# Newiz430/CellSegmentation

Hardware: AMD Instinct MI355X
Metric: tiles/sec fwd+bwd (ResNet-50 MIL, 299x299) (higher is better)
Workload: dtype bf16; 1 GPU; ResNet-50 tile classifier (train_tile.py --scratch semantics: fwd + CE + full bwd + Adam), bag=64 tiles of 299x299x3 per GPU, freeze_bn=True; tiles_per_gpu=64, parallelism=dp1

## Files before the change

### cellsegmentation_amd/csrc/conv_v2.hip

```cpp
#include "cs_common.h"
#include <stdio.h>
#include <stdlib.h>
#include <utility>

namespace {

typedef int i32x4 __attribute__((ext_vector_type(4)));
typedef unsigned u32x4 __attribute__((ext_vector_type(4)));
constexpr unsigned OOB = 0x80000000u;

struct C2Params {
    const void* src;
    const void* wpk;
    void* dst;
    const float* shift;
    const void* residual;
    unsigned char* bits_out;
    const unsigned char* bits_in;
    float* slab;
    int act;
    int SH, SW, SC, NS;
    int DH, DW, NOUT;
    int Wp, Hp, PW, PH;
    int LW;
    int TH, TWl, tiles_x, tiles_y;
    unsigned n_tiles;
    int stride;
    int gather, GH, GWp;
    unsigned tap_sh[9];
    int lin;
    unsigned chunk_bytes;
    int add_stride, AH, AW;
    unsigned mg_dw, sh_dw, mg_dh, sh_dh, mg_wp, sh_wp, mg_hp, sh_hp;
    int NCC;
    int n_ntiles;
    unsigned M;
    unsigned src_bytes;
    unsigned pix_bytes;
    unsigned wpk_bytes;
};

__device__ __forceinline__ unsigned udivm(unsigned n, unsigned mg, unsigned sh) { return __umulhi(n, mg) >> sh; }

__device__ __forceinline__ i32x4 make_rsrc(const void* base, unsigned bytes) {
    const unsigned long long a = (unsigned long long)base;
    i32x4 r;
    r.x = (int)(unsigned)a;
    r.y = (int)((unsigned)(a >> 32) & 0xffffu);
    r.z = (int)bytes;
    r.w = 0x00020000;
    return r;
}
__device__ __forceinline__ unsigned lds_off(const void* p) { return (unsigned)(size_t)(__attribute__((address_space(3))) const unsigned char*)p; }

template <int N> __device__ __forceinline__ void wait_vm() { asm volatile("s_waitcnt vmcnt(%0)" ::"n"(N)); }
template <int N> __device__ __forceinline__ void wait_vm_mem() { asm volatile("s_waitcnt vmcnt(%0)" ::"n"(N) : "memory"); }
__device__ __forceinline__ void raw_barrier() { asm volatile("s_barrier" ::: "memory"); }

__device__ __forceinline__ void dma_block(const i32x4& rsrc, unsigned lds_dst, unsigned voff, unsigned soff) {
    unsigned tmp;
    asm volatile(
        "s_mov_b32 m0, %1\n\t"
        "s_add_u32 %0, %4, 64\n\t"
        "buffer_load_dwordx4 %2, %3, %4 offen lds\n\t"
        "s_add_u32 m0, %1, 0x400\n\t"
// ... 143 lines not shown
    const unsigned wds[4] = {o.x, o.y, o.z, o.w};
    unsigned t = 0;
#pragma unroll
    for (int i = 0; i < 4; ++i) {
        const unsigned a = ((wds[i] & 0x7fff7fffu) + 0x7fff7fffu) & ~wds[i];
        t |= ((a >> 15) & 0x10001u) << (2 * i);
    }
    return (t | (t >> 15)) & 0xffu;
}
__device__ __forceinline__ unsigned nz_bits8(const uint4& o) {
    const unsigned wds[4] = {o.x, o.y, o.z, o.w};
    const unsigned ones = 0x00010001u;
    unsigned u = 0;
#pragma unroll
    for (int i = 0; i < 4; ++i) {
        unsigned t;
        asm("v_pk_min_u16 %0, %1, %2" : "=v"(t) : "v"(wds[i]), "s"(ones));
        u |= t << (2 * i);
    }
    return (u | (u >> 15)) & 0xffu;
}
struct TileOffs {
    static constexpr bool kPreset = false;
    static constexpr unsigned NONE = 0x7fffff00u;
    unsigned rb, mr, bb, br;
    __device__ __forceinline__ void set(unsigned base, bool ok, unsigned nout, unsigned n_w, unsigned piece, unsigned M) {
        const unsigned lane = threadIdx.x & 63;
        const bool live = ok && base != 0xffffffffu;
        const unsigned m = base + (lane >> 2);
        mr = live ? m : NONE;
        rb = (m * nout + n_w + 8u * piece) * 2u;
        const unsigned mbit = m + 16u * (lane & 1u);
        br = (live && !(lane & 2u)) ? mbit : NONE;
        bb = ((n_w >> 5) * M + mbit) * 4u;
    }
    __device__ __forceinline__ unsigned row(unsigned M, unsigned nout, int i, int q) const {
        const unsigned d = (unsigned)(2 * i + q);
        return mr + 16u * d < M ? rb + d * (32u * nout) : OOB;
    }
    __device__ __forceinline__ unsigned bit(unsigned M, unsigned nout, int i) const {
        return br + 32u * (unsigned)i < M ? bb + (unsigned)i * 128u : OOB;
    }
};
template <int TM> struct TileOffs2D {
    static constexpr bool kPreset = true;
    unsigned ro[TM][2], bo[TM];
    __device__ __forceinline__ void set2d(unsigned n, unsigned y0, unsigned x0, unsigned dh, unsigned dw, unsigned twl, unsigned j0, bool alive,
                                          unsigned nout, unsigned n_w, unsigned piece, unsigned M) {
        const unsigned lane = threadIdx.x & 63, tw1 = (1u << twl) - 1u;
#pragma unroll
        for (int i = 0; i < TM; ++i) {
#pragma unroll
            for (int q = 0; q < 2; ++q) {
                const unsigned j = j0 + 32u * i + 16u * q + (lane >> 2);
                const unsigned y = y0 + (j >> twl), x = x0 + (j & tw1);
                const unsigned m = (n * dh + y) * dw + x;
                ro[i][q] = (alive && y < dh && x < dw) ? (m * nout + n_w + 8u * piece) * 2u : OOB;
            }
            const unsigned jb = j0 + 32u * i + (lane >> 2) + 16u * (lane & 1u);
            const unsigned yb = y0 + (jb >> twl), xb = x0 + (jb & tw1);
            const unsigned mb = (n * dh + yb) * dw + xb;
            bo[i] = (alive && !(lane & 2u) && yb < dh && xb < dw) ? ((n_w >> 5) * M + mb) * 4u : OOB;
        }
    }
    __device__ __forceinline__ unsigned row(unsigned, unsigned, int i, int q) const { return ro[i][q]; }
    __device__ __forceinline__ unsigned bit(unsigned, unsigned, int i) const { return bo[i]; }
};
__device__ __forceinline__ uint4 keep_bits8(const uint4& o, unsigned b) {
    unsigned wds[4] = {o.x, o.y, o.z, o.w};
#pragma unroll
    for (int i = 0; i < 4; ++i) {
        const unsigned m = (b >> (2 * i));
        wds[i] &= (m & 1u) * 0xffffu + (m & 2u) * 0x7fff8000u;
    }
    return make_uint4(wds[0], wds[1], wds[2], wds[3]);
}


__device__ __forceinline__ unsigned compact_add_off(const C2Params& p, unsigned m, unsigned n_w, unsigned piece) {
    const unsigned yall = udivm(m, p.mg_dw, p.sh_dw);
    const unsigned x = m - yall * (unsigned)p.DW;
    const unsigned n = udivm(yall, p.mg_dh, p.sh_dh);
    const unsigned y = yall - n * (unsigned)p.DH;
    const unsigned mc = (n * (unsigned)p.AH + (y >> 1)) * (unsigned)p.AW + (x >> 1);
    return (m < p.M && !((x | y) & 1u)) ? (mc * (unsigned)p.NOUT + n_w + 8u * piece) * 2u : OOB;
}
template <bool DG> __device__ __forceinline__ void load_shift(const C2Params& p, int n_w, bool alive, float (&sh)[16]) {
    const int lane = threadIdx.x & 63;
    const int hh = lane >> 5;
#pragma unroll
// ... 72 lines not shown
    }
    __device__ __forceinline__ unsigned acc_lds(int j) const {
        const int lane = threadIdx.x & 63;
        return scr + (unsigned)(lane & 31) * EPI_ROW + (unsigned)(2 * j + (lane >> 5)) * 16u;
    }

    __device__ __forceinline__ unsigned res_off(int i, int q) const {
        if constexpr (TO::kPreset) return to.row(p.M, (unsigned)p.NOUT, i, q);
        else {
            if (p.add_stride <= 1) return to.row(p.M, (unsigned)p.NOUT, i, q);
            const unsigned lane = threadIdx.x & 63;
            const unsigned m = to.mr + 16u * (unsigned)(2 * i + q);
            const unsigned yall = udivm(m, p.mg_dw, p.sh_dw);
            const unsigned x = m - yall * (unsigned)p.DW;
            const unsigned n = udivm(yall, p.mg_dh, p.sh_dh);
            const unsigned y = yall - n * (unsigned)p.DH;
            const unsigned mc = (n * (unsigned)p.AH + (y >> 1)) * (unsigned)p.AW + (x >> 1);
            return (m < p.M && !((x | y) & 1u)) ? (mc * (unsigned)p.NOUT + (unsigned)n_w + 8u * (lane & 3u)) * 2u : OOB;
        }
    }

    __device__ __forceinline__ void prefetch() {
        const int lane = threadIdx.x & 63;
        const unsigned out_bytes = p.M * (unsigned)p.NOUT * 2u;
        if constexpr (!TO::kPreset) to.set(m0w, alive, (unsigned)p.NOUT, (unsigned)n_w, (unsigned)(lane & 3), p.M);
        r_dst = __builtin_amdgcn_make_buffer_rsrc(p.dst, 0, out_bytes, 0x00020000);
        r_res = __builtin_amdgcn_make_buffer_rsrc(const_cast<void*>(p.residual), 0,
                                                  !p.residual ? 0u : p.add_stride == 2 ? (unsigned)(p.NS * p.AH * p.AW * p.NOUT) * 2u : out_bytes, 0x00020000);
        r_bin = __builtin_amdgcn_make_buffer_rsrc(const_cast<unsigned char*>(p.bits_in), 0, p.bits_in ? out_bytes >> 4 : 0u, 0x00020000);
        r_bout = __builtin_amdgcn_make_buffer_rsrc(p.bits_out, 0, p.bits_out ? out_bytes >> 4 : 0u, 0x00020000);
        load_shift<DG>(p, n_w, alive, sh);
#pragma unroll
        for (int i = 0; i < TM; ++i) {
            if constexpr (PRE_RES) {
                rr[i][0] = __builtin_bit_cast(uint4, __builtin_amdgcn_raw_buffer_load_b128(r_res, res_off(i, 0), 0, 0));
                rr[i][1] = __builtin_bit_cast(uint4, __builtin_amdgcn_raw_buffer_load_b128(r_res, res_off(i, 1), 0, 0));
            }
            if constexpr (DG) mb[i] = __builtin_amdgcn_raw_buffer_load_b32(r_bin, to.bit(p.M, (unsigned)p.NOUT, i), 0, 0);
        }
    }

    template <int I> __device__ __forceinline__ void operator()(const f32x16& acc) {
        const int lane = threadIdx.x & 63;
        const unsigned piece = (unsigned)(lane & 3);
        float v[16];
#pragma unroll
        for (int r = 0; r < 16; ++r) v[r] = DG ? acc[r] : acc[r] + sh[r];
// ... 35 lines not shown
        if (!DG && p.bits_out) {
            unsigned w0, w1;
            plane_dwords(o0, o1, p.act == CS_ACT_RELU, piece, w0, w1);
            __builtin_amdgcn_raw_buffer_store_b32((lane & 1) ? w1 : w0, r_bout, to.bit(p.M, (unsigned)p.NOUT, I), 0, 0);
        }
    }

    __device__ __forceinline__ void finish() {
        if (!DG || !p.slab || !alive) return;
        const int lane = threadIdx.x & 63;
#pragma unroll
        for (int k = 0; k < 8; ++k) {
#pragma unroll
            for (int off = 32; off >= 4; off >>= 1) s1[k] += __shfl_xor(s1[k], off, 64);
        }
        if (lane < 4) {
            float* dst = p.slab + (size_t)slab_row * 2 * p.NOUT + n_w + 8 * lane;
            *reinterpret_cast<float4*>(dst) = make_float4(s1[0], s1[1], s1[2], s1[3]);
            *reinterpret_cast<float4*>(dst + 4) = make_float4(s1[4], s1[5], s1[6], s1[7]);
        }
    }
};

template <int NTAP, int SK, int TM, int WM, int WN, int NBW, bool DG, bool T2D = false>
__global__ __launch_bounds__(256, 2) __attribute__((amdgpu_num_vgpr(50))) void conv2_halo_kernel(C2Params p) {
    static_assert(WM * WN == 4 && NTAP % 3 == 0 && NBW <= 8, "layout");
    constexpr int BM = WM * TM * 32, BN = WN * 32;
    constexpr unsigned STAGE = NBW * 4 * 2048;
    extern __shared__ __attribute__((aligned(16))) unsigned char smem[];

    const int tid = threadIdx.x, lane = tid & 63;
    const int wave = __builtin_amdgcn_readfirstlane(tid >> 6);
    const int wm = wave / WN, wn = wave % WN;
    const int l31 = lane & 31, hh = lane >> 5;

    const WgTile wg(p);
    const unsigned mtile = wg.mtile, m0 = mtile * BM;
    if (T2D ? mtile >= p.n_tiles : m0 >= p.M) return;
    const int n_w = wg.n_w(p, BN, wn);
    const bool alive = n_w < p.NOUT;

    using TOffs = std::conditional_t<T2D, TileOffs2D<TM>, TileOffs>;
    Epilogue<TM, (NBW == 8), DG, TOffs> epi(p, m0 + (unsigned)(wm * TM * 32), n_w, mtile * WM + wm, alive, 0u);
    unsigned qb[TM];
    unsigned voff[NBW];
    if constexpr (T2D) {
        const unsigned per_img = (unsigned)(p.tiles_y * p.tiles_x);
        const unsigned n = mtile / per_img, tr = mtile - n * per_img;
        const unsigned ty = tr / (unsigned)p.tiles_x, tx = tr - ty * (unsigned)p.tiles_x;
        const unsigned y0 = ty * (unsigned)p.TH, x0 = tx << p.TWl;
        const unsigned j0 = (unsigned)(wm * TM * 32);
#pragma unroll
        for (int i = 0; i < TM; ++i) {
            const unsigned j = j0 + 32u * i + (unsigned)l31;
            qb[i] = (j >> p.TWl) * (unsigned)p.LW + (j & ((1u << p.TWl) - 1u));
        }
        const unsigned win_rows = (unsigned)(p.TH + (NTAP / SK) - 1) * (unsigned)p.LW;
#pragma unroll
        for (int j = 0; j < NBW; ++j) {
            const unsigned l = 16u * (unsigned)(wave + 4 * j) + (unsigned)(lane & 15);
            const unsigned ly = udivm(l, p.mg_wp, p.sh_wp);
            const unsigned lx = l - ly * (unsigned)p.LW;
            const int sy = (int)(y0 + ly) - p.PH, sx = (int)(x0 + lx) - p.PW;
            const bool real = l < win_rows && (unsigned)sy < (unsigned)p.SH && (unsigned)sx < (unsigned)p.SW;
            const unsigned pix = (n * (unsigned)p.SH + (unsigned)sy) * (unsigned)p.SW + (unsigned)sx;
            voff[j] = real ? pix * p.pix_bytes + (unsigned)(lane >> 4) * 16u : OOB;
        }
        epi.to.set2d(n, y0, x0, (unsigned)p.DH, (unsigned)p.DW, (unsigned)p.TWl, j0, alive, (unsigned)p.NOUT, (unsigned)n_w, (unsigned)(lane & 3), p.M);
    } else {
        auto pos0 = [&](unsigned m) -> unsigned {
            const unsigned yall = udivm(m, p.mg_dw, p.sh_dw);
            const unsigned x = m - yall * (unsigned)p.DW;
            const unsigned n = udivm(yall, p.mg_dh, p.sh_dh);
            const unsigned y = yall - n * (unsigned)p.DH;
            return (n * (unsigned)p.Hp + y) * (unsigned)p.Wp + x;
        };
        const unsigned Lmin = pos0(m0);
        const unsigned m0w = m0 + (unsigned)(wm * TM * 32);
#pragma unroll
        for (int i = 0; i < TM; ++i) {
            unsigned m = m0w + 32u * i + (unsigned)l31;
            if (m > p.M - 1) m = p.M - 1;
            qb[i] = pos0(m) - Lmin;
        }
#pragma unroll
        for (int j = 0; j < NBW; ++j) {
            const unsigned L = Lmin + 16u * (unsigned)(wave + 4 * j) + (unsigned)(lane & 15);
            const unsigned row = udivm(L, p.mg_wp, p.sh_wp);
            const unsigned col = L - row * (unsigned)p.Wp;
            const unsigned n = udivm(row, p.mg_hp, p.sh_hp);
            const unsigned ry = row - n * (unsigned)p.Hp;
            const bool real = col >= (unsigned)p.PW && ry >= (unsigned)p.PH && n < (unsigned)p.NS;
            const unsigned pix = (n * (unsigned)p.SH + (ry - (unsigned)p.PH)) * (unsigned)p.SW + (col - (unsigned)p.PW);
            voff[j] = real ? pix * p.pix_bytes + (unsigned)(lane >> 4) * 16u : OOB;
        }
    }
    const i32x4 rsrc_a = make_rsrc(p.src, p.src_bytes);
    const i32x4 rsrc_b = make_rsrc(p.wpk, p.wpk_bytes);
    const unsigned bvoff = alive ? (unsigned)lane * 16u : OOB;
    unsigned wsoff = (unsigned)(n_w >> 5) * (unsigned)p.NCC * (unsigned)(NTAP * 4096);
    const unsigned smem_base = lds_off(smem);

    static_assert(TM >= 2 && TM <= 4, "the register map of the main loop holds up to 4 pixel tiles per wave");
    epi.prefetch();
    own_registers();
    vzero_seq(std::make_integer_sequence<int, 16 * TM>{});
    const unsigned hhb = (unsigned)hh * 256u;
    const unsigned cf0 = 0xf0u;

#pragma unroll
    for (int j = 0; j < NBW; ++j) dma_block(rsrc_a, smem_base + (unsigned)(wave + 4 * j) * 2048u, voff[j], 0u);
    bload4<0>(rsrc_b, bvoff, wsoff); wsoff += 4096u;
    bload4<1>(rsrc_b, bvoff, wsoff); wsoff += 4096u;
    wait_vm<8>();
    raw_barrier();

    unsigned nxt_soff = 128u;

    auto tap = [&]<int T, bool ODD, bool HN>() {
        constexpr int CUR = T % 3, NX2 = (T + 2) % 3;
        constexpr bool has1 = HN || (T + 1 < NTAP);
        constexpr bool has2 = HN || (T + 2 < NTAP);
        constexpr bool LAST = T == NTAP - 1;
        constexpr int D0 = (HN && !LAST && T < NBW) ? 2 : 0;
        constexpr int D1 = (HN && !LAST && T >= 1 && T - 1 < NBW) ? 2 : 0;
        constexpr int D2 = (HN && !LAST && T >= 2 && T - 2 < NBW) ? 2 : 0;
        constexpr unsigned CUR_STAGE = ODD ? STAGE : 0u, NXT_STAGE = ODD ? 0u : STAGE;
        if constexpr (has2) {
            bload4<NX2>(rsrc_b, bvoff, wsoff);
            wsoff += 4096u;
        }
        if constexpr (D0) dma_block(rsrc_a, smem_base + NXT_STAGE + (unsigned)(wave + 4 * T) * 2048u, voff[T < NBW ? T : 0], nxt_soff);
        wait_vm<(has1 ? 4 : 0) + (has2 ? 4 : 0) + D0 + D1 + D2>();
        const unsigned sh_cur = (unsigned)(T / SK) * (unsigned)p.LW + (unsigned)(T % SK);
        const unsigned sh_next = (unsigned)((T + 1) / SK) * (unsigned)p.LW + (unsigned)((T + 1) % SK);
        if constexpr (T == NTAP - 1 && !HN) epi.scr = smem_base + NXT_STAGE + (unsigned)wave * EPI_WAVE;
        tap_mfma<TM, CUR, T & 1, CUR_STAGE, CUR_STAGE, T == 0, T != NTAP - 1, false, (T == NTAP - 1 && !HN)>(qb[0], qb[1], qb[2 % TM], qb[3 % TM], sh_cur, sh_next,
                                                                                                          hhb, cf0, epi);
    };
    auto chunk = [&]<bool ODD, bool HN>() {
        [&]<int... Ts>(std::integer_sequence<int, Ts...>) { (tap.template operator()<Ts, ODD, HN>(), ...); }(std::make_integer_sequence<int, NTAP>{});
    };

    if constexpr (NBW == 8) {
        chunk.template operator()<false, false>();
    } else {
        for (int cc = 0; cc < p.NCC; cc += 2) {
            if (cc) { raw_barrier(); nxt_soff += 128u; }
            if (cc + 1 < p.NCC) chunk.template operator()<false, true>();
            else chunk.template operator()<false, false>();
            if (cc + 1 < p.NCC) {
                raw_barrier();
                nxt_soff += 128u;
                if (cc + 2 < p.NCC) chunk.template operator()<true, true>();
                else chunk.template operator()<true, false>();
            }
        }
    }
    epi.finish();
}


constexpr int W_TMP = 100, W_AD = 104, W_AF = 120, W_B = 184, W_ACC = 128, W_NSLOT = 18;

template <int N, typename F> __device__ __forceinline__ void for_n(F&& f) {
    [&]<int... Is>(std::integer_sequence<int, Is...>) { (f.template operator()<Is>(), ...); }(std::make_integer_sequence<int, N>{});
}
template <int REG> __device__ __forceinline__ void azero() { asm volatile("v_accvgpr_write_b32 a[%c0], 0" ::"i"(REG)); }
template <int REG> __device__ __forceinline__ float aget() {
    float x;
    asm volatile("v_accvgpr_read_b32 %0, a[%c1]" : "=v"(x) : "i"(REG));
    return x;
}
template <int I> __device__ __forceinline__ f32x16 acc_read_w() {
    f32x16 d;
    [&]<int... Rs>(std::integer_sequence<int, Rs...>) { ((d[Rs] = aget<W_ACC + 16 * I + Rs>()), ...); }(std::make_integer_sequence<int, 16>{});
    return d;
}
// ... 618 lines not shown
    magic((unsigned)p.LW, p.mg_wp, p.sh_wp);
    magic((unsigned)Hp, p.mg_hp, p.sh_hp);
    if (t2d) {
        p.TH = 8; p.TWl = 4;
        p.tiles_x = cs_ceil_div(DW, 16); p.tiles_y = cs_ceil_div(DH, 8);
        const long long nt = (long long)g->N * p.tiles_x * p.tiles_y;
        if (nt >= (1ll << 28)) return false;
        p.n_tiles = (unsigned)nt;
    }
    p.NCC = ncc;
    p.M = (unsigned)M;
    p.src_bytes = (unsigned)src_bytes;
    p.pix_bytes = (unsigned)SC * 2u;
    const unsigned long long wbytes = (unsigned long long)cs_ceil_div(NOUT, 32) * 32 * g->R * g->S * (unsigned long long)SC * 2ull;
    if (wbytes >= 0x80000000ull) return false;
    p.wpk_bytes = (unsigned)wbytes;
    const int BM = cfg != 2 ? 32 * tm : 256, BN = cfg != 2 ? 128 : 64;
    p.n_ntiles = cs_ceil_div(NOUT, BN);
    pl.cfg = cfg; pl.nbw = nbw; pl.ncc = ncc; pl.tm = cfg != 2 ? tm : 4;
    pl.t2d = t2d;
    pl.rows = t2d ? (int)p.n_tiles : cs_ceil_div(M, BM) * (cfg != 2 ? 1 : 2);
    return true;
}
unsigned ring_groups(unsigned n_mt, unsigned n_ntiles, unsigned long long* cost_out) {
    const unsigned cap = (n_mt + 7u) / 8u * 8u;
    unsigned best = 8u;
    unsigned long long best_cost = ~0ull, best_tiles = 0;
    for (unsigned g = 8u; g <= cap; g += 8u) {
        const unsigned long long rounds = ((unsigned long long)g * n_ntiles + 511ull) / 512ull;
        const unsigned long long cost = rounds * ((n_mt + g - 1u) / g) * 16ull + rounds;
        if (cost <= best_cost) { best_cost = cost; best = g; best_tiles = rounds * ((n_mt + g - 1u) / g); }
    }
    if (cost_out) *cost_out = best_tiles;
    return best;
}

bool plan_gemm(const CsConvGeom* g, int dgrad, C2Plan& pl) {
    if (g->groups > 1) return false;
    if (g->R != 1 || g->S != 1 || g->pad != 0 || g->stride < 1) return false;
    const bool compact = dgrad && g->stride != 1;
    if (compact && g->stride != 2) return false;
    const int SC = dgrad ? g->K : g->C, NOUT = dgrad ? g->C : g->K;
    const int SH = dgrad ? g->P : g->H, SW = dgrad ? g->Q : g->W;
    const int DH = dgrad ? (compact ? g->P : g->H) : g->P, DW = dgrad ? (compact ? g->Q : g->W) : g->Q;
    if (SC % 64 || NOUT % 64 || DH < 1 || DW < 1) return false;
    if (!dgrad && g->stride > 1 && (DH < 2 || DW < 2)) return false;
// ... 138 lines not shown
        const unsigned n_mt = (unsigned)cs_ceil_div(p.M, 256);
        dim3 grid(((n_mt + 7) / 8) * 8 * (unsigned)p.n_ntiles);
        cs_set_variant_(DG ? "conv2_halo_kernel<9,3,4,2,2,8,true,false>" : "conv2_halo_kernel<9,3,4,2,2,8,false,false>");
        if (!allow_lds(conv2_halo_kernel<9, 3, 4, 2, 2, 8, DG>, 8 * 8192 + EPI_LDS)) return CS_ERR_LAUNCH;
        hipLaunchKernelGGL((conv2_halo_kernel<9, 3, 4, 2, 2, 8, DG>), grid, dim3(256), 8 * 8192 + EPI_LDS, st, p);
        CS_LAUNCH_CHECK();
        return CS_OK;
    }
    const int two = pl.ncc > 1;
    if (pl.t2d) return launch_cfg1<4, 3, DG, true>(p, st, two);
#define CS_HALO_TM(TM_)                                         \
    switch (pl.nbw) {                                           \
        case 3: return launch_cfg1<TM_, 3, DG>(p, st, two);     \
        case 4: return launch_cfg1<TM_, 4, DG>(p, st, two);     \
        case 5: return launch_cfg1<TM_, 5, DG>(p, st, two);     \
        default: return launch_cfg1<TM_, 8, DG>(p, st, 0);      \
    }
    if (pl.tm == 2) { CS_HALO_TM(2) }
    if (pl.tm == 3) { CS_HALO_TM(3) }
    CS_HALO_TM(4)
#undef CS_HALO_TM
}

}

static bool plan_any(const CsConvGeom* g, int dgrad, C2Plan& pl) { return plan_halo(g, dgrad, pl) || plan_gemm(g, dgrad, pl); }
static int launch_any(const C2Plan& pl, hipStream_t st, bool dg) {
    if (dg) return pl.cfg <= 3 ? launch_halo<true>(pl, st) : launch_gemm<true>(pl, st);
    return pl.cfg <= 3 ? launch_halo<false>(pl, st) : launch_gemm<false>(pl, st);
}

extern "C" int cs_conv2d_packed_supported(const CsConvGeom* g, int dgrad) {
    if (!g) return 0;
    C2Plan pl;
    return plan_any(g, dgrad, pl) ? 1 : 0;
}

extern "C" size_t cs_conv2d_packed_weight_bytes(const CsConvGeom* g, int dgrad) {
    if (!g) return 0;
    const int rows = dgrad ? g->C : g->K, cols = dgrad ? g->K : g->C;
    return (size_t)cs_ceil_div(rows, 32) * 32 * g->R * g->S * (size_t)cols * 2;
}

extern "C" int cs_pack_conv_weights(const CsConvGeom* g, int dgrad, const void* w_staged, void* w_packed, void* stream) {
    CS_CHECK_ARG(g && w_staged && w_packed, "pack_conv_weights: NULL argument");
    const int rows = dgrad ? g->C : g->K, cols = dgrad ? g->K : g->C;
    CS_CHECK_ARG(cols % 64 == 0 && rows % 8 == 0, "pack_conv_weights: contraction channels must be a multiple of 64");
    const long long total = (long long)cs_ceil_div(rows, 32) * (cols / 64) * g->R * g->S * 4 * 64;
    long long nb = (total + 255) / 256;
    if (nb > 8192) nb = 8192;
// ... 13 lines not shown
                                    void* y, uint8_t* positive_bits, void* stream) {
    CS_CHECK_ARG(g && x && w_packed && y, "conv2d_fwd_packed: NULL tensor");
    CS_CHECK_ARG(act == CS_ACT_NONE || act == CS_ACT_RELU, "conv2d_fwd_packed: activation must be none or ReLU");
    C2Plan pl;
    if (!plan_any(g, 0, pl)) {
        cs_set_error_("conv2d_fwd_packed: geometry not served by the packed-operand kernel (ask cs_conv2d_packed_supported first)");
        return CS_ERR_UNSUPPORTED;
    }
    pl.p.src = x; pl.p.wpk = w_packed; pl.p.dst = y;
    pl.p.shift = shift; pl.p.residual = residual; pl.p.act = act;
    pl.p.bits_out = positive_bits;
    return launch_any(pl, reinterpret_cast<hipStream_t>(stream), false);
}

extern "C" int cs_conv2d_dgrad_packed(const CsConvGeom* g, const void* dy, const void* w_packed, const void* add, int add_stride,
                                      const uint8_t* mask_bits, void* dx, float* partial_rows, void* stream) {
    CS_CHECK_ARG(g && dy && w_packed && dx, "conv2d_dgrad_packed: NULL tensor");
    CS_CHECK_ARG(add_stride == 1 || (add_stride == 2 && add), "conv2d_dgrad_packed: add_stride is 1, or 2 with a compact add operand");
    C2Plan pl;
    if (!plan_any(g, 1, pl)) {
        cs_set_error_("conv2d_dgrad_packed: geometry not served by the packed-operand kernel (ask cs_conv2d_packed_supported first)");
        return CS_ERR_UNSUPPORTED;
    }
    if (g->stride != 1)
        CS_CHECK_ARG(!add && !mask_bits && !partial_rows,
                     "conv2d_dgrad_packed: a strided 1x1 data gradient is written in compact [N][P][Q][C] form, without add / mask / column sums");
    if (add_stride == 2) {
        CS_CHECK_ARG(pl.cfg >= 6 && pl.p.DH >= 2 && pl.p.DW >= 2, "conv2d_dgrad_packed: a strided add operand is served by the 1x1 kernels only");
        pl.p.add_stride = 2;
        pl.p.AH = (pl.p.DH + 1) / 2;
        pl.p.AW = (pl.p.DW + 1) / 2;
    }
    pl.p.src = dy; pl.p.wpk = w_packed; pl.p.dst = dx;
    pl.p.residual = add; pl.p.act = CS_ACT_NONE;
    pl.p.bits_in = mask_bits;
    pl.p.slab = partial_rows;
    return launch_any(pl, reinterpret_cast<hipStream_t>(stream), true);
}

extern "C" int cs_stem_fwd_packed(int N, int H, int W, int K, const void* x_pair, const void* w_packed, const float* shift, int act, void* y,
                                  uint8_t* positive_bits, void* stream) {
    CS_CHECK_ARG(x_pair && w_packed && y && N > 0 && H >= 7 && W >= 7, "stem_fwd_packed: bad arguments");
    CS_CHECK_ARG(K == 64, "stem_fwd_packed: 64 output channels (the stem of every ResNet / ResNeXt of model/resnet.py)");
    CS_CHECK_ARG(act == CS_ACT_NONE || act == CS_ACT_RELU, "stem_fwd_packed: activation must be none or ReLU");
    const int P = (H - 1) / 2 + 1, Q = (W - 1) / 2 + 1, Wh = (W + 1) / 2;
    const long long M = (long long)N * P * Q;
    const unsigned long long src_bytes = (unsigned long long)N * H * Wh * 16ull;
    CS_CHECK_ARG(P >= 2 && Q >= 2 && M < (1ll << 31) - 512 && src_bytes < 0x80000000ull, "stem_fwd_packed: extents out of range");
    C2Plan pl;
    C2Params& p = pl.p;
    p = C2Params{};
// ... 19 lines not shown
```

### cellsegmentation_amd/engine.py

```python
from collections import namedtuple
from types import SimpleNamespace

import torch

from . import _capture
from . import kernels as K

ACT_NONE, ACT_RELU, ACT_SILU = K.CS_ACT_NONE, K.CS_ACT_RELU, K.CS_ACT_SILU

PACKED = True
PACKED_TRAIN_BN = True


class ConvUnit:
    kind = "conv"

    def __init__(self, name, conv, bn, act, src, dst, res=None):
        self.name, self.conv, self.bn, self.act = name, conv, bn, act
        self.src, self.dst, self.res = src, dst, res
        self.grouped = conv.groups != 1
        if self.grouped:
            cg = conv.in_channels // conv.groups
            if conv.in_channels != conv.out_channels or conv.in_channels % 64 != 0 or 64 % cg != 0 or conv.bias is not None:
                raise NotImplementedError(f"{name}: grouped convolution needs C == K, C % 64 == 0, (C/groups) | 64, no bias "
# ... 304 lines not shown
    return (not u.grouped and u.res is None and c.in_channels <= 3 and c.kernel_size == (7, 7)
            and c.stride == (2, 2) and c.padding == (3, 3))


def _stem_takes_nchw(plan, dtype):
    if not (dtype == torch.bfloat16 and len(plan.inputs) == 1 and plan.units):
        return False
    u = plan.units[0]
    return (_is_paired_stem(u) and u.conv.in_channels == 3 and u.src == plan.inputs[0]
            and plan.consumers.get(u.src, 0) == 1)


def _packed_flags(plan, u, geom, dtype, need_bwd, batch_stats, bits, bn_train=False):
    if not PACKED or u.grouped or u.act not in (ACT_NONE, ACT_RELU):
        return False, False
    if batch_stats:
        if not (PACKED_TRAIN_BN and geom.R == 3 and geom.S == 3 and geom.stride == 1 and min(geom.C, geom.K) >= 128):
            return False, False
        pkf = K.packed_supported(geom, dtype, dgrad=False)
        pkb = bool(need_bwd) and K.packed_supported(geom, dtype, dgrad=True) and geom.C % 32 == 0
        return pkf, pkb
    pkf = K.packed_supported(geom, dtype, dgrad=False)
    pkb = bool(need_bwd) and K.packed_supported(geom, dtype, dgrad=True) and (u.src not in plan.relu_slots or u.src in bits)
    if pkb and geom.stride != 1:
        pkb = _compact_partner(plan, u, geom, dtype, bits, bn_train) is not None
    return pkf, pkb


def _compact_partner(plan, u, geom, dtype, bits, bn_train=False):
    others = [(i, v) for i, v in enumerate(plan.units) if v is not u and v.kind == "conv" and v.src == u.src]
    if len(others) != 1 or plan.consumers.get(u.src, 0) != 2:
        return None
    iv, v = others[0]
    iu = plan.units.index(u)
    c = v.conv
    if iv > iu or v.grouped or v.act not in (ACT_NONE, ACT_RELU) or c.kernel_size != (1, 1) or c.stride != (1, 1) or c.padding != (0, 0):
        return None
    if not PACKED or _bn_uses_batch_stats(v.bn, bn_train):
        return None
    if u.src in plan.relu_slots and u.src not in bits:
        return None
    gv = K.make_geom(geom.N, geom.H, geom.W, geom.C, K.pad_channels(c.out_channels), 1, 1, 1, 0)
    if not K.packed_supported(gv, dtype, dgrad=True):
        return None
    return v


# ... 341 lines not shown
        w = conv.weight.detach() if want_bn else None
        scale, rstd = (None, None) if a.train else (a.st.scale, a.st.rstd)
        mean = u.bn.running_mean if want_bn else None
        if u.grouped:
            K.wgrad_finalize_grouped(raw, w, scale, rstd, mean, gsum, dw, dgamma=dgamma, dbeta=dbeta, dot=dot)
        else:
            K.wgrad_finalize(raw, w, scale, rstd, mean, gsum, conv.in_channels, dw, dbias=dbias, dgamma=dgamma, dbeta=dbeta, dot=dot)
        if self.need(ui, "weight"):
            self.emit(ui, "weight", dw)
        if want_b:
            self.emit(ui, "bias", dbias)
        if want_bn:
            self.emit_bn(ui, dgamma, dbeta)

    def conv_dgrad(self, u, a, x, dz):
        geom, st = a.geom, a.st
        self.left[u.src] -= 1
        final = self.left[u.src] == 0
        pending = self.grads.pop(u.src, None)
        mask = x if (u.src in self.plan.relu_slots and final) else None
        mbits = self.bits.get(u.src) if mask is not None else None
        if mbits is not None:
            mask = None
        if st.bwd_packed and geom.stride != 1:
            if final or pending is not None:
                raise RuntimeError(f"{u.name}: compact strided data gradient out of order (it must be the first contribution)")
            return K.conv_dgrad_packed(geom, dz, st.w_chwk)
        if st.bwd_packed:
            if mask is not None and a.train:
                mbits, mask = K.positive_bits(mask), None
            if mask is not None:
                raise RuntimeError(f"{u.name}: packed data-gradient operand staged but the ReLU mask is not a bit tensor")
            if not final:
                return K.conv_dgrad_packed(geom, dz, st.w_chwk, add=pending, mask_bits=mbits)
            dx, self.gsum_cache[u.src] = K.conv_dgrad_packed(geom, dz, st.w_chwk, add=pending, mask_bits=mbits, want_colsum=True)
            return dx
        if isinstance(pending, K.CompactGrad):
            raise RuntimeError(f"{u.name}: a compact gradient reached a data gradient that cannot add it")
        if not final:
            return K.conv_dgrad(geom, dz, st.w_chwk, add=pending, mask=mask, grouped=u.grouped, mask_bits=mbits)
        cs = self.take(geom.C) if (geom.stride != 1 or u.grouped) else None
        dx, self.gsum_cache[u.src] = K.conv_dgrad(geom, dz, st.w_chwk, add=pending, mask=mask, colsum=cs, grouped=u.grouped,
                                                  defer_colsum=True, mask_bits=mbits)
        return dx


def backward(plan, state, grad_feeds, param_needs, requires, use_tr_read=True):
# ... 49 lines not shown
```

### cellsegmentation_amd/kernels.py

```python
import ctypes

import torch

from . import _lib
from ._lib import (CS_ACT_NONE, CS_ACT_RELU, CS_ACT_SIGMOID, CS_ACT_SILU, CS_BF16, CS_BN_BWD_FROZEN, CS_BN_BWD_OWN_RELU, CS_F32,
                   CsConvGeom)


def _code(dtype):
    if dtype == torch.float32:
        return CS_F32
    if dtype == torch.bfloat16:
        return CS_BF16
    raise TypeError(f"unsupported activation dtype {dtype}; use torch.float32 or torch.bfloat16")


def _f32(*tensors):
    for t in tensors:
        if t.dtype != torch.float32:
            raise TypeError(f"this kernel reads torch.float32 only, got {t.dtype}; cast on the way in (functional.py does)")


def chunk(dtype):
    return 4 if dtype == torch.float32 else 8
# ... 235 lines not shown
        out = torch.empty((n,), dtype=torch.bfloat16, device=w_staged.device)
    _lib.check(lib.cs_pack_conv_weights(ctypes.byref(geom), 1 if dgrad else 0, _p(w_staged), _p(out), _stream()), "pack_conv_weights")
    return out


def conv_fwd_packed(geom, x, w_packed, shift=None, residual=None, act=CS_ACT_NONE, want_bits=False, out=None):
    y = out if out is not None else torch.empty((geom.N, geom.P, geom.Q, geom.K), dtype=x.dtype, device=x.device)
    bits = torch.empty((geom.N, geom.P, geom.Q, geom.K // 8), dtype=torch.uint8, device=x.device) if want_bits else None
    lib = _lib.load()
    _lib.check(_timed("fwd", geom, x.dtype, lambda: lib.cs_conv2d_fwd_packed(
        ctypes.byref(geom), _p(x), _p(w_packed), _p(shift), _p(residual), act, _p(y), _p(bits), _stream()),
        extra_tensors=int(residual is not None) + (1.0 / 16 if want_bits else 0.0)), "conv2d_fwd_packed")
    return (y, bits) if want_bits else y


class CompactGrad:

    def __init__(self, t, stride):
        self.t, self.stride = t, stride


def conv_dgrad_packed(geom, dy, w_packed, add=None, mask_bits=None, want_colsum=False):
    lib = _lib.load()
    if geom.stride != 1:
        if add is not None or mask_bits is not None or want_colsum:
            raise ValueError("conv_dgrad_packed: a strided 1x1 data gradient is compact -- no add, mask or column sums")
        dxc = torch.empty((geom.N, geom.P, geom.Q, geom.C), dtype=dy.dtype, device=dy.device)
        _lib.check(_timed("dgrad", geom, dy.dtype, lambda: lib.cs_conv2d_dgrad_packed(
            ctypes.byref(geom), _p(dy), _p(w_packed), None, 1, None, _p(dxc), None, _stream()), extra_tensors=-0.75), "conv2d_dgrad_packed")
        return CompactGrad(dxc, geom.stride)
    add_stride = 1
    if isinstance(add, CompactGrad):
        add_stride, add = add.stride, add.t
        if tuple(add.shape) != (geom.N, (geom.H + 1) // 2, (geom.W + 1) // 2, geom.C):
            raise ValueError("conv_dgrad_packed: compact add operand of another destination")
    dx = torch.empty((geom.N, geom.H, geom.W, geom.C), dtype=dy.dtype, device=dy.device)
    rows = lib.cs_conv2d_packed_partial_rows(ctypes.byref(geom), 1) if want_colsum else 0
    ws = torch.empty((rows, 2 * geom.C), dtype=torch.float32, device=dy.device) if want_colsum else None
    _lib.check(_timed("dgrad", geom, dy.dtype, lambda: lib.cs_conv2d_dgrad_packed(
        ctypes.byref(geom), _p(dy), _p(w_packed), _p(add), add_stride, _p(mask_bits), _p(dx), _p(ws), _stream()),
        extra_tensors=(int(add is not None) if add_stride == 1 else 0.25) + (1.0 / 16 if mask_bits is not None else 0.0)), "conv2d_dgrad_packed")
    if want_colsum:
        return dx, PartialColsum(ws, rows, geom.C)
    return dx


def is_stem_geom(geom):
# ... 1214 lines not shown
```

Baseline: 9210 tiles/s.

## Add parity-class packed dgrad kernel for stride-2 3x3 convolutions

Adds a packed-operand halo data-gradient path for stride-2 3x3 convolutions. The output is split into four parity classes (even/odd row and column), and each class runs only the 1, 2, 2 or 4 weight taps that reach it, so the kernel avoids the zero-inserted upsampled gradient. A new tile-offset struct scatters each class's rows into the full-resolution destination. The engine now routes these layers to the packed path when the source has a single consumer, in place of the old generic path. This adds kernel complexity, an extra LDS scratch region and per-class epilogues, and it only covers the three stride-2 3x3 layers in ResNet-50.

Measured after the change: 9275 tiles/s (median of 6 runs). About the same (+0.7%).

```diff
diff --git a/cellsegmentation_amd/csrc/conv_v2.hip b/cellsegmentation_amd/csrc/conv_v2.hip
--- a/cellsegmentation_amd/csrc/conv_v2.hip
+++ b/cellsegmentation_amd/csrc/conv_v2.hip
@@ -38,9 +38,12 @@
     unsigned src_bytes;
     unsigned pix_bytes;
     unsigned wpk_bytes;
+    int FH, FW;
+    unsigned Mdst;
 };
 
 __device__ __forceinline__ unsigned udivm(unsigned n, unsigned mg, unsigned sh) { return __umulhi(n, mg) >> sh; }
+__device__ __forceinline__ unsigned udivm1(unsigned n, unsigned d, unsigned mg, unsigned sh) { return d == 1u ? n : udivm(n, mg, sh); }
 
 __device__ __forceinline__ i32x4 make_rsrc(const void* base, unsigned bytes) {
     const unsigned long long a = (unsigned long long)base;
@@ -230,6 +233,7 @@
 }
 struct TileOffs {
     static constexpr bool kPreset = false;
+    static __device__ __forceinline__ unsigned rows(const C2Params& p) { return p.M; }
     static constexpr unsigned NONE = 0x7fffff00u;
     unsigned rb, mr, bb, br;
     __device__ __forceinline__ void set(unsigned base, bool ok, unsigned nout, unsigned n_w, unsigned piece, unsigned M) {
@@ -252,6 +256,7 @@
 };
 template <int TM> struct TileOffs2D {
     static constexpr bool kPreset = true;
+    static __device__ __forceinline__ unsigned rows(const C2Params& p) { return p.M; }
     unsigned ro[TM][2], bo[TM];
     __device__ __forceinline__ void set2d(unsigned n, unsigned y0, unsigned x0, unsigned dh, unsigned dw, unsigned twl, unsigned j0, bool alive,
                                           unsigned nout, unsigned n_w, unsigned piece, unsigned M) {
@@ -274,6 +279,35 @@
     __device__ __forceinline__ unsigned row(unsigned, unsigned, int i, int q) const { return ro[i][q]; }
     __device__ __forceinline__ unsigned bit(unsigned, unsigned, int i) const { return bo[i]; }
 };
+template <int TM> struct TileOffsS2 {
+    static constexpr bool kPreset = true;
+    static __device__ __forceinline__ unsigned rows(const C2Params& p) { return p.Mdst; }
+    unsigned ro[TM][2], bo[TM];
+    static __device__ __forceinline__ unsigned dst_row(const C2Params& p, unsigned j, unsigned a, unsigned b) {
+        const unsigned yall = udivm1(j, (unsigned)p.DW, p.mg_dw, p.sh_dw);
+        const unsigned x = 2u * (j - yall * (unsigned)p.DW) + b;
+        const unsigned n = udivm1(yall, (unsigned)p.DH, p.mg_dh, p.sh_dh);
+        const unsigned y = 2u * (yall - n * (unsigned)p.DH) + a;
+        return (j < p.M && y < (unsigned)p.FH && x < (unsigned)p.FW) ? (n * (unsigned)p.FH + y) * (unsigned)p.FW + x : 0xffffffffu;
+    }
+    __device__ __forceinline__ void set_s2(const C2Params& p, unsigned m0w, bool alive, unsigned n_w, unsigned piece, unsigned a, unsigned b) {
+        const unsigned lane = threadIdx.x & 63;
+#pragma unroll
+        for (int i = 0; i < TM; ++i) {
+#pragma unroll
+            for (int q = 0; q < 2; ++q) {
+                const unsigned m = dst_row(p, m0w + 32u * i + 16u * q + (lane >> 2), a, b);
+                ro[i][q] = (alive && m != 0xffffffffu) ? (m * (unsigned)p.NOUT + n_w + 8u * piece) * 2u : OOB;
+            }
+            const unsigned mb = dst_row(p, m0w + 32u * i + (lane >> 2) + 16u * (lane & 1u), a, b);
+            bo[i] = (alive && !(lane & 2u) && mb != 0xffffffffu) ? ((n_w >> 5) * p.Mdst + mb) * 4u : OOB;
+        }
+    }
+    __device__ __forceinline__ unsigned row(unsigned, unsigned, int i, int q) const { return ro[i][q]; }
+    __device__ __forceinline__ unsigned bit(unsigned, unsigned, int i) const { return bo[i]; }
+};
+constexpr unsigned long long S2_TAP_IDS = 0x8620007100530004ull;
+constexpr unsigned S2_NTAPS = 0x4221u;
 __device__ __forceinline__ uint4 keep_bits8(const uint4& o, unsigned b) {
     unsigned wds[4] = {o.x, o.y, o.z, o.w};
 #pragma unroll
@@ -392,7 +426,7 @@
 
     __device__ __forceinline__ void prefetch() {
         const int lane = threadIdx.x & 63;
-        const unsigned out_bytes = p.M * (unsigned)p.NOUT * 2u;
+        const unsigned out_bytes = TO::rows(p) * (unsigned)p.NOUT * 2u;
         if constexpr (!TO::kPreset) to.set(m0w, alive, (unsigned)p.NOUT, (unsigned)n_w, (unsigned)(lane & 3), p.M);
         r_dst = __builtin_amdgcn_make_buffer_rsrc(p.dst, 0, out_bytes, 0x00020000);
         r_res = __builtin_amdgcn_make_buffer_rsrc(const_cast<void*>(p.residual), 0,
@@ -474,9 +508,10 @@
     }
 };
 
-template <int NTAP, int SK, int TM, int WM, int WN, int NBW, bool DG, bool T2D = false>
+template <int NTAP, int SK, int TM, int WM, int WN, int NBW, bool DG, bool T2D = false, int S2 = 0>
 __global__ __launch_bounds__(256, 2) __attribute__((amdgpu_num_vgpr(50))) void conv2_halo_kernel(C2Params p) {
     static_assert(WM * WN == 4 && NTAP % 3 == 0 && NBW <= 8, "layout");
+    static_assert(!S2 || (NTAP == 9 && DG && !T2D && WM == 1 && NBW <= 4), "parity classes: 9 taps of the packed operand, two stages + the exchange scratch");
     constexpr int BM = WM * TM * 32, BN = WN * 32;
     constexpr unsigned STAGE = NBW * 4 * 2048;
     extern __shared__ __attribute__((aligned(16))) unsigned char smem[];
@@ -492,7 +527,7 @@
     const int n_w = wg.n_w(p, BN, wn);
     const bool alive = n_w < p.NOUT;
 
-    using TOffs = std::conditional_t<T2D, TileOffs2D<TM>, TileOffs>;
+    using TOffs = std::conditional_t<T2D, TileOffs2D<TM>, std::conditional_t<S2 != 0, TileOffsS2<TM>, TileOffs>>;
     Epilogue<TM, (NBW == 8), DG, TOffs> epi(p, m0 + (unsigned)(wm * TM * 32), n_w, mtile * WM + wm, alive, 0u);
     unsigned qb[TM];
     unsigned voff[NBW];
@@ -521,20 +556,25 @@
         epi.to.set2d(n, y0, x0, (unsigned)p.DH, (unsigned)p.DW, (unsigned)p.TWl, j0, alive, (unsigned)p.NOUT, (unsigned)n_w, (unsigned)(lane & 3), p.M);
     } else {
         auto pos0 = [&](unsigned m) -> unsigned {
-            const unsigned yall = udivm(m, p.mg_dw, p.sh_dw);
+            unsigned yall, n;
+            if constexpr (S2) yall = udivm1(m, (unsigned)p.DW, p.mg_dw, p.sh_dw);
+            else yall = udivm(m, p.mg_dw, p.sh_dw);
             const unsigned x = m - yall * (unsigned)p.DW;
-            const unsigned n = udivm(yall, p.mg_dh, p.sh_dh);
+            if constexpr (S2) n = udivm1(yall, (unsigned)p.DH, p.mg_dh, p.sh_dh);
+            else n = udivm(yall, p.mg_dh, p.sh_dh);
             const unsigned y = yall - n * (unsigned)p.DH;
             return (n * (unsigned)p.Hp + y) * (unsigned)p.Wp + x;
         };
-        const unsigned Lmin = pos0(m0);
+        const unsigned L0 = pos0(m0);
+        const unsigned Lmin = S2 ? L0 + (unsigned)p.Wp + 1u : L0;
         const unsigned m0w = m0 + (unsigned)(wm * TM * 32);
 #pragma unroll
         for (int i = 0; i < TM; ++i) {
             unsigned m = m0w + 32u * i + (unsigned)l31;
             if (m > p.M - 1) m = p.M - 1;
-            qb[i] = pos0(m) - Lmin;
-        }
+            qb[i] = pos0(m) - L0;
+        }
+        if constexpr (S2) epi.to.set_s2(p, m0w, alive, (unsigned)n_w, (unsigned)(lane & 3), 0u, 0u);
 #pragma unroll
         for (int j = 0; j < NBW; ++j) {
             const unsigned L = Lmin + 16u * (unsigned)(wave + 4 * j) + (unsigned)(lane & 15);
@@ -560,52 +600,141 @@
     const unsigned hhb = (unsigned)hh * 256u;
     const unsigned cf0 = 0xf0u;
 
-#pragma unroll
-    for (int j = 0; j < NBW; ++j) dma_block(rsrc_a, smem_base + (unsigned)(wave + 4 * j) * 2048u, voff[j], 0u);
-    bload4<0>(rsrc_b, bvoff, wsoff); wsoff += 4096u;
-    bload4<1>(rsrc_b, bvoff, wsoff); wsoff += 4096u;
-    wait_vm<8>();
-    raw_barrier();
-
-    unsigned nxt_soff = 128u;
-
-    auto tap = [&]<int T, bool ODD, bool HN>() {
-        constexpr int CUR = T % 3, NX2 = (T + 2) % 3;
-        constexpr bool has1 = HN || (T + 1 < NTAP);
-        constexpr bool has2 = HN || (T + 2 < NTAP);
-        constexpr bool LAST = T == NTAP - 1;
-        constexpr int D0 = (HN && !LAST && T < NBW) ? 2 : 0;
-        constexpr int D1 = (HN && !LAST && T >= 1 && T - 1 < NBW) ? 2 : 0;
-        constexpr int D2 = (HN && !LAST && T >= 2 && T - 2 < NBW) ? 2 : 0;
-        constexpr unsigned CUR_STAGE = ODD ? STAGE : 0u, NXT_STAGE = ODD ? 0u : STAGE;
-        if constexpr (has2) {
-            bload4<NX2>(rsrc_b, bvoff, wsoff);
-            wsoff += 4096u;
-        }
-        if constexpr (D0) dma_block(rsrc_a, smem_base + NXT_STAGE + (unsigned)(wave + 4 * T) * 2048u, voff[T < NBW ? T : 0], nxt_soff);
-        wait_vm<(has1 ? 4 : 0) + (has2 ? 4 : 0) + D0 + D1 + D2>();
-        const unsigned sh_cur = (unsigned)(T / SK) * (unsigned)p.LW + (unsigned)(T % SK);
-        const unsigned sh_next = (unsigned)((T + 1) / SK) * (unsigned)p.LW + (unsigned)((T + 1) % SK);
-        if constexpr (T == NTAP - 1 && !HN) epi.scr = smem_base + NXT_STAGE + (unsigned)wave * EPI_WAVE;
-        tap_mfma<TM, CUR, T & 1, CUR_STAGE, CUR_STAGE, T == 0, T != NTAP - 1, false, (T == NTAP - 1 && !HN)>(qb[0], qb[1], qb[2 % TM], qb[3 % TM], sh_cur, sh_next,
-                                                                                                          hhb, cf0, epi);
-    };
-    auto chunk = [&]<bool ODD, bool HN>() {
-        [&]<int... Ts>(std::integer_sequence<int, Ts...>) { (tap.template operator()<Ts, ODD, HN>(), ...); }(std::make_integer_sequence<int, NTAP>{});
-    };
-
-    if constexpr (NBW == 8) {
-        chunk.template operator()<false, false>();
+    if constexpr (S2) {
+        constexpr bool RES = S2 == 2;
+        epi.scr = smem_base + 2u * STAGE + (unsigned)wave * EPI_WAVE;
+        unsigned wq_k = 0u, wq_c = 0u, wq_t = 0u;
+        auto wnext = [&]() -> unsigned {
+            const unsigned k = wq_k & 3u;
+            const unsigned id = (unsigned)(S2_TAP_IDS >> (16u * k + 4u * wq_t)) & 15u;
+            const unsigned off = wq_k < 4u ? wsoff + (wq_c * 9u + id) * 4096u : p.wpk_bytes;
+            if (++wq_t == ((S2_NTAPS >> (4u * k)) & 15u)) {
+                wq_t = 0u;
+                if (++wq_c == (unsigned)p.NCC) { wq_c = 0u; ++wq_k; }
+            }
+            return off;
+        };
+#pragma unroll
+        for (int j = 0; j < NBW; ++j) dma_block(rsrc_a, smem_base + (unsigned)(wave + 4 * j) * 2048u, voff[j], 0u);
+        if constexpr (RES) {
+#pragma unroll
+            for (int j = 0; j < NBW; ++j) dma_block(rsrc_a, smem_base + STAGE + (unsigned)(wave + 4 * j) * 2048u, voff[j], p.NCC > 1 ? 128u : 0u);
+        }
+        bload4<0>(rsrc_b, bvoff, wnext());
+        bload4<1>(rsrc_b, bvoff, wnext());
+        wait_vm<8>();
+        raw_barrier();
+
+        unsigned nxt_soff = 0u;
+        auto tap = [&]<int C_, int T, int PH, bool ODD>() {
+            constexpr int NT = (1 + (C_ >> 1)) * (1 + (C_ & 1)), SKC = 1 + (C_ & 1);
+            constexpr int CUR = (T + PH) % 3, NX2 = (T + PH + 2) % 3;
+            constexpr unsigned CUR_STAGE = ODD ? STAGE : 0u, NXT_STAGE = ODD ? 0u : STAGE;
+            if constexpr (T == 0 && !RES) {
+#pragma unroll
+                for (int j = 0; j < NBW; ++j) dma_block(rsrc_a, smem_base + NXT_STAGE + (unsigned)(wave + 4 * j) * 2048u, voff[j], nxt_soff);
+            }
+            bload4<NX2>(rsrc_b, bvoff, wnext());
+            wait_vm<8 + (!RES && T <= 1 ? 2 * NBW : 0)>();
+            const unsigned sh_cur = (unsigned)(T / SKC) * (unsigned)p.LW + (unsigned)(T % SKC);
+            const unsigned sh_next = (unsigned)((T + 1) / SKC) * (unsigned)p.LW + (unsigned)((T + 1) % SKC);
+            tap_mfma<TM, CUR, T & 1, CUR_STAGE, CUR_STAGE, T == 0, T != NT - 1, false, false>(qb[0], qb[1], qb[2 % TM], qb[3 % TM], sh_cur, sh_next, hhb, cf0);
+        };
+        unsigned ph = 0u, odd = 0u;
+        auto chunk = [&]<int C_>() {
+            constexpr int NT = (1 + (C_ >> 1)) * (1 + (C_ & 1));
+            auto body = [&]<int PH, bool ODD>() {
+                [&]<int... Ts>(std::integer_sequence<int, Ts...>) { (tap.template operator()<C_, Ts, PH, ODD>(), ...); }(std::make_integer_sequence<int, NT>{});
+            };
+            switch (ph * 2u + odd) {
+                case 0: body.template operator()<0, false>(); break;
+                case 1: body.template operator()<0, true>(); break;
+                case 2: body.template operator()<1, false>(); break;
+                case 3: body.template operator()<1, true>(); break;
+                case 4: body.template operator()<2, false>(); break;
+                default: body.template operator()<2, true>(); break;
+            }
+            if constexpr (NT <= 2 && !RES) wait_vm<4 * NT>();
+            ph = (ph + (unsigned)NT) % 3u;
+            odd ^= 1u;
+        };
+        const unsigned n_mt = (p.M + (unsigned)BM - 1u) / (unsigned)BM;
+        auto cls = [&]<int C_>() {
+            if constexpr (C_ > 0) {
+                epi.to.set_s2(p, m0, alive, (unsigned)n_w, (unsigned)(lane & 3), (unsigned)(C_ >> 1), (unsigned)(C_ & 1));
+                epi.slab_row = (unsigned)C_ * n_mt + mtile;
+                epi.prefetch();
+            }
+            for (int c = 0; c < p.NCC; ++c) {
+                nxt_soff = c + 1 < p.NCC ? (unsigned)(c + 1) * 128u : 0u;
+                chunk.template operator()<C_>();
+                if (!RES && c + 1 < p.NCC) raw_barrier();
+            }
+            asm volatile("s_nop 15\n\ts_nop 3");
+            for_tiles<TM>([&]<int i>() {
+                f32x16 d;
+                acc_tile<i>(d, std::make_integer_sequence<int, 16>{});
+                epi.template operator()<i>(d);
+            });
+            if constexpr (C_ < 3) {
+                epi.finish();
+                vzero_seq(std::make_integer_sequence<int, 16 * TM>{});
+                if constexpr (!RES) raw_barrier();
+            }
+        };
+        cls.template operator()<0>();
+        cls.template operator()<1>();
+        cls.template operator()<2>();
+        cls.template operator()<3>();
+        wait_vm<0>();
     } else {
-        for (int cc = 0; cc < p.NCC; cc += 2) {
-            if (cc) { raw_barrier(); nxt_soff += 128u; }
-            if (cc + 1 < p.NCC) chunk.template operator()<false, true>();
-            else chunk.template operator()<false, false>();
-            if (cc + 1 < p.NCC) {
-                raw_barrier();
-                nxt_soff += 128u;
-                if (cc + 2 < p.NCC) chunk.template operator()<true, true>();
-                else chunk.template operator()<true, false>();
+#pragma unroll
+        for (int j = 0; j < NBW; ++j) dma_block(rsrc_a, smem_base + (unsigned)(wave + 4 * j) * 2048u, voff[j], 0u);
+        bload4<0>(rsrc_b, bvoff, wsoff); wsoff += 4096u;
+        bload4<1>(rsrc_b, bvoff, wsoff); wsoff += 4096u;
+        wait_vm<8>();
+        raw_barrier();
+
+        unsigned nxt_soff = 128u;
+
+        auto tap = [&]<int T, bool ODD, bool HN>() {
+            constexpr int CUR = T % 3, NX2 = (T + 2) % 3;
+            constexpr bool has1 = HN || (T + 1 < NTAP);
+            constexpr bool has2 = HN || (T + 2 < NTAP);
+            constexpr bool LAST = T == NTAP - 1;
+            constexpr int D0 = (HN && !LAST && T < NBW) ? 2 : 0;
+            constexpr int D1 = (HN && !LAST && T >= 1 && T - 1 < NBW) ? 2 : 0;
+            constexpr int D2 = (HN && !LAST && T >= 2 && T - 2 < NBW) ? 2 : 0;
+            constexpr unsigned CUR_STAGE = ODD ? STAGE : 0u, NXT_STAGE = ODD ? 0u : STAGE;
+            if constexpr (has2) {
+                bload4<NX2>(rsrc_b, bvoff, wsoff);
+                wsoff += 4096u;
+            }
+            if constexpr (D0) dma_block(rsrc_a, smem_base + NXT_STAGE + (unsigned)(wave + 4 * T) * 2048u, voff[T < NBW ? T : 0], nxt_soff);
+            wait_vm<(has1 ? 4 : 0) + (has2 ? 4 : 0) + D0 + D1 + D2>();
+            const unsigned sh_cur = (unsigned)(T / SK) * (unsigned)p.LW + (unsigned)(T % SK);
+            const unsigned sh_next = (unsigned)((T + 1) / SK) * (unsigned)p.LW + (unsigned)((T + 1) % SK);
+            if constexpr (T == NTAP - 1 && !HN) epi.scr = smem_base + NXT_STAGE + (unsigned)wave * EPI_WAVE;
+            tap_mfma<TM, CUR, T & 1, CUR_STAGE, CUR_STAGE, T == 0, T != NTAP - 1, false, (T == NTAP - 1 && !HN)>(qb[0], qb[1], qb[2 % TM], qb[3 % TM], sh_cur, sh_next,
+                                                                                                              hhb, cf0, epi);
+        };
+        auto chunk = [&]<bool ODD, bool HN>() {
+            [&]<int... Ts>(std::integer_sequence<int, Ts...>) { (tap.template operator()<Ts, ODD, HN>(), ...); }(std::make_integer_sequence<int, NTAP>{});
+        };
+
+        if constexpr (NBW == 8) {
+            chunk.template operator()<false, false>();
+        } else {
+            for (int cc = 0; cc < p.NCC; cc += 2) {
+                if (cc) { raw_barrier(); nxt_soff += 128u; }
+                if (cc + 1 < p.NCC) chunk.template operator()<false, true>();
+                else chunk.template operator()<false, false>();
+                if (cc + 1 < p.NCC) {
+                    raw_barrier();
+                    nxt_soff += 128u;
+                    if (cc + 2 < p.NCC) chunk.template operator()<true, true>();
+                    else chunk.template operator()<true, false>();
+                }
             }
         }
     }
@@ -1270,6 +1399,46 @@
     pl.rows = t2d ? (int)p.n_tiles : cs_ceil_div(M, BM) * (cfg != 2 ? 1 : 2);
     return true;
 }
+bool plan_halo_s2(const CsConvGeom* g, int dgrad, C2Plan& pl) {
+    if (!dgrad || g->groups > 1 || g->R != 3 || g->S != 3 || g->stride != 2 || g->pad != 1) return false;
+    const int SC = g->K, NOUT = g->C, SH = g->P, SW = g->Q, FH = g->H, FW = g->W;
+    if (NOUT % 128 || SC % 64 || FH < 2 || FW < 2 || SH != (FH + 1) / 2 || SW != (FW + 1) / 2 || g->N < 1) return false;
+    const long long M = (long long)g->N * SH * SW, Mdst = (long long)g->N * FH * FW;
+    const unsigned long long src_bytes = (unsigned long long)g->N * SH * SW * SC * 2ull;
+    const unsigned long long wbytes = (unsigned long long)NOUT * 9ull * (unsigned long long)SC * 2ull;
+    const int Wp = SW + 1, Hp = SH + 1;
+    if ((unsigned long long)Mdst * NOUT * 2ull >= 0x80000000ull || src_bytes >= 0x80000000ull || wbytes >= 0x80000000ull) return false;
+    if ((long long)g->N * Hp * Wp + 4096 >= (1ll << 31)) return false;
+    const long long bm = M < 128 ? M : 128;
+    const long long span = (bm - 1) + cs_ceil_div(bm - 1, SW) + (long long)cs_ceil_div(bm - 1, (long long)SH * SW) * Wp;
+    const int nb = (int)((span + Wp + 1 + 1 + 63) / 64);
+    if (nb > 4) return false;
+    const long long cus = cs_device_cus_();
+    if (cs_ceil_div(M, 128) * (long long)(NOUT / 128) < cus && cs_ceil_div(Mdst, 64) * (long long)(NOUT / 128) >= cus) return false;
+    C2Params& p = pl.p;
+    p = C2Params{};
+    p.SH = SH; p.SW = SW; p.SC = SC; p.NS = g->N;
+    p.DH = SH; p.DW = SW; p.NOUT = NOUT;
+    p.Wp = Wp; p.Hp = Hp; p.PW = 1; p.PH = 1;
+    p.stride = 1;
+    p.LW = Wp;
+    p.chunk_bytes = 128u;
+    if (SW >= 2) magic((unsigned)SW, p.mg_dw, p.sh_dw);
+    if (SH >= 2) magic((unsigned)SH, p.mg_dh, p.sh_dh);
+    magic((unsigned)Wp, p.mg_wp, p.sh_wp);
+    magic((unsigned)Hp, p.mg_hp, p.sh_hp);
+    p.FH = FH; p.FW = FW;
+    p.Mdst = (unsigned)Mdst;
+    p.NCC = SC / 64;
+    p.M = (unsigned)M;
+    p.src_bytes = (unsigned)src_bytes;
+    p.pix_bytes = (unsigned)SC * 2u;
+    p.wpk_bytes = (unsigned)wbytes;
+    p.n_ntiles = NOUT / 128;
+    pl.cfg = 9; pl.nbw = nb < 3 ? 3 : nb; pl.ncc = p.NCC; pl.tm = 4; pl.t2d = 0;
+    pl.rows = 4 * cs_ceil_div(M, 128);
+    return true;
+}
 unsigned ring_groups(unsigned n_mt, unsigned n_ntiles, unsigned long long* cost_out) {
     const unsigned cap = (n_mt + 7u) / 8u * 8u;
     unsigned best = 8u;
@@ -1454,10 +1623,30 @@
 #undef CS_HALO_TM
 }
 
-}
-
-static bool plan_any(const CsConvGeom* g, int dgrad, C2Plan& pl) { return plan_halo(g, dgrad, pl) || plan_gemm(g, dgrad, pl); }
+template <int NBW, int S2>
+int launch_s2(const C2Params& p, hipStream_t st) {
+    const unsigned n_mt = (unsigned)cs_ceil_div(p.M, 128);
+    dim3 grid(((n_mt + 7) / 8) * 8 * (unsigned)p.n_ntiles);
+    const size_t lds = (size_t)NBW * 8192 * 2 + EPI_LDS;
+    auto fn = conv2_halo_kernel<9, 3, 4, 1, 4, NBW, true, false, S2>;
+    if (!allow_lds(fn, lds)) return CS_ERR_LAUNCH;
+    char name[64];
+    snprintf(name, sizeof(name), "conv2_halo_kernel<9,3,4,1,4,%d,true,false,%d>", NBW, S2);
+    cs_set_variant_(name);
+    hipLaunchKernelGGL(fn, grid, dim3(256), lds, st, p);
+    CS_LAUNCH_CHECK();
+    return CS_OK;
+}
+int launch_halo_s2(const C2Plan& pl, hipStream_t st) {
+    if (pl.ncc <= 2) return pl.nbw == 3 ? launch_s2<3, 2>(pl.p, st) : launch_s2<4, 2>(pl.p, st);
+    return pl.nbw == 3 ? launch_s2<3, 1>(pl.p, st) : launch_s2<4, 1>(pl.p, st);
+}
+
+}
+
+static bool plan_any(const CsConvGeom* g, int dgrad, C2Plan& pl) { return plan_halo(g, dgrad, pl) || plan_halo_s2(g, dgrad, pl) || plan_gemm(g, dgrad, pl); }
 static int launch_any(const C2Plan& pl, hipStream_t st, bool dg) {
+    if (pl.cfg == 9) return launch_halo_s2(pl, st);
     if (dg) return pl.cfg <= 3 ? launch_halo<true>(pl, st) : launch_gemm<true>(pl, st);
     return pl.cfg <= 3 ? launch_halo<false>(pl, st) : launch_gemm<false>(pl, st);
 }
@@ -1517,11 +1706,11 @@
         cs_set_error_("conv2d_dgrad_packed: geometry not served by the packed-operand kernel (ask cs_conv2d_packed_supported first)");
         return CS_ERR_UNSUPPORTED;
     }
-    if (g->stride != 1)
+    if (g->stride != 1 && pl.cfg != 9)
         CS_CHECK_ARG(!add && !mask_bits && !partial_rows,
                      "conv2d_dgrad_packed: a strided 1x1 data gradient is written in compact [N][P][Q][C] form, without add / mask / column sums");
     if (add_stride == 2) {
-        CS_CHECK_ARG(pl.cfg >= 6 && pl.p.DH >= 2 && pl.p.DW >= 2, "conv2d_dgrad_packed: a strided add operand is served by the 1x1 kernels only");
+        CS_CHECK_ARG(pl.cfg >= 6 && pl.cfg <= 8 && pl.p.DH >= 2 && pl.p.DW >= 2, "conv2d_dgrad_packed: a strided add operand is served by the 1x1 kernels only");
         pl.p.add_stride = 2;
         pl.p.AH = (pl.p.DH + 1) / 2;
         pl.p.AW = (pl.p.DW + 1) / 2;
diff --git a/cellsegmentation_amd/engine.py b/cellsegmentation_amd/engine.py
--- a/cellsegmentation_amd/engine.py
+++ b/cellsegmentation_amd/engine.py
@@ -350,7 +350,9 @@
         return pkf, pkb
     pkf = K.packed_supported(geom, dtype, dgrad=False)
     pkb = bool(need_bwd) and K.packed_supported(geom, dtype, dgrad=True) and (u.src not in plan.relu_slots or u.src in bits)
-    if pkb and geom.stride != 1:
+    if pkb and geom.stride != 1 and (geom.R, geom.S) != (1, 1):
+        pkb = plan.consumers.get(u.src, 0) == 1
+    elif pkb and geom.stride != 1:
         pkb = _compact_partner(plan, u, geom, dtype, bits, bn_train) is not None
     return pkf, pkb
 
@@ -738,7 +740,7 @@
         mbits = self.bits.get(u.src) if mask is not None else None
         if mbits is not None:
             mask = None
-        if st.bwd_packed and geom.stride != 1:
+        if st.bwd_packed and geom.stride != 1 and (geom.R, geom.S) == (1, 1):
             if final or pending is not None:
                 raise RuntimeError(f"{u.name}: compact strided data gradient out of order (it must be the first contribution)")
             return K.conv_dgrad_packed(geom, dz, st.w_chwk)
diff --git a/cellsegmentation_amd/kernels.py b/cellsegmentation_amd/kernels.py
--- a/cellsegmentation_amd/kernels.py
+++ b/cellsegmentation_amd/kernels.py
@@ -281,7 +281,9 @@
 
 def conv_dgrad_packed(geom, dy, w_packed, add=None, mask_bits=None, want_colsum=False):
     lib = _lib.load()
-    if geom.stride != 1:
+    if geom.stride != 1 and isinstance(add, CompactGrad):
+        raise ValueError("conv_dgrad_packed: a strided data gradient cannot add a compact operand")
+    if geom.stride != 1 and geom.R == 1 and geom.S == 1:
         if add is not None or mask_bits is not None or want_colsum:
             raise ValueError("conv_dgrad_packed: a strided 1x1 data gradient is compact -- no add, mask or column sums")
         dxc = torch.empty((geom.N, geom.P, geom.Q, geom.C), dtype=dy.dtype, device=dy.device)
```
